# apple/swift-homomorphic-encryption

Measured on NVIDIA H100. Metric: BFV ct*ct mults/sec at N=8192, 4 coefficient moduli, higher is better.
Workload: dtype u64

## Files before the change

### swift-homomorphic-encryption_b200/csrc/context.cu

```cuda
#include "context.hpp"

#include <cuda_runtime.h>

#include <cmath>
#include <cstdlib>
#include <cstring>

#include "hostmath.hpp"
#include "ntt_fast.cuh"

namespace hecuda {
using namespace host;


static void fill_barrett(u64 p, u64 &mu1, u64 &mu_hi, u64 &mu_lo) {
    mu1 = (u64)(((u128)1 << 64) / p);
    u128 mu = (p & (p - 1)) == 0 ? ((u128)1 << (128 - (bit_length(p) - 1))) : (~(u128)0) / p;
    mu_hi = (u64)(mu >> 64);
    mu_lo = (u64)mu;
}

static bool build_slot(HostSlot &hs, u64 p, int64_t n, int logn, u64 t, u64 floor_w, std::vector<ulonglong2> &tw,
                       std::vector<ulonglong2> &itw, std::string &err) {
    if (!is_prime(p) || (p - 1) % (2 * (u64)n) != 0) {
// ... 99 lines not shown
    for (u64 qi : c->q)
        if (t >= qi) { err = "invalidEncryptionParameters: plaintext modulus must be below every coefficient modulus"; delete c; return nullptr; }
    c->bsk = smallest_ntt_primes(word_bits - 3, L + 1, (u64)n);
    if ((int)c->bsk.size() != L + 1) { err = "notEnoughPrimes for Bsk"; delete c; return nullptr; }
    for (u64 b : c->bsk)
        for (int i = 0; i < nmod; ++i)
            if (b == coeff_moduli[i]) { err = "coprimeModuli: coefficient modulus collides with the BEHZ base"; delete c; return nullptr; }

    c->aux = c->bsk;
    {
        const char *env = std::getenv("HECUDA_AUX_BASE");
        const bool want_fast = !(env && std::string(env) == "reference");
        const int widths[2] = {30, 55};
        double log_q = 0;
        for (u64 v : c->q) log_q += std::log2((double)v);
        const double log_n = (double)c->logn, log_t = std::log2((double)t);
        for (int wi = 0; wi < 2 && want_fast && c->aux == c->bsk && word_bits == 64; ++wi) {
            std::vector<u64> cand = widths[wi] == 55 ? smallest_ntt_primes(55, L + 1 + nmod, 1ull << 31)
                                                     : smallest_ntt_primes(widths[wi], L + 1 + nmod, (u64)n);
            std::vector<u64> pick;
            for (u64 v : cand) {
                bool used = false;
                for (int i = 0; i < nmod; ++i) used |= coeff_moduli[i] == v;
                if (!used && (int)pick.size() < L + 1) pick.push_back(v);
            }
            double log_aux = 0, log_aux_l = 0;
            for (size_t j = 0; j < pick.size(); ++j) {
                log_aux += std::log2((double)pick[j]);
                if ((int)j < L) log_aux_l += std::log2((double)pick[j]);
            }
            const bool enough = (int)pick.size() == L + 1 && log_aux >= log_q + log_n + 4 &&
                                log_aux_l + std::log2((double)pick.back()) >= log_t + log_n + log_q + 5;
            if (enough) c->aux = pick;
        }
    }
    c->aux_is_reference = c->aux == c->bsk;

    c->simd = is_prime(t) && (t - 1) % (2 * (u64)n) == 0;
    const int nslots = (c->aux_is_reference ? 2 * L + 2 : 3 * L + 3) + (c->simd ? 1 : 0);
    c->slots.resize(nslots);
    std::vector<u64> slot_mod(nslots);
    if (c->simd) slot_mod[c->slot_t()] = t;
    for (int i = 0; i < L; ++i) slot_mod[c->slot_q(i)] = c->q[i];
    for (int j = 0; j <= L; ++j) slot_mod[c->slot_bsk(j)] = c->bsk[j];
    slot_mod[c->slot_ks()] = c->q_ks;
    if (!c->aux_is_reference)
        for (int j = 0; j <= L; ++j) slot_mod[c->slot_aux(j)] = c->aux[j];
    const size_t table_bytes = sizeof(ulonglong2) * (size_t)n;
    const bool fast = c->logn >= fast::kMinLogN && c->logn <= fast::kMaxLogN;
    const bool split = c->logn == fast::kSplitLogN;
    const int half_logn = c->logn - 1;
    const int64_t half_n = n / 2;
    const int threads = (int)((split ? half_n : n) / 16);
    const size_t tr_bytes = (fast || split) ? sizeof(ulonglong2) * (size_t)15 * threads : 0;
    const size_t half_bytes = sizeof(ulonglong2) * (size_t)half_n;
    const size_t slot_bytes = 2 * table_bytes + (split ? 2 * (2 * half_bytes + 2 * tr_bytes) : 2 * tr_bytes);
    if (cudaMalloc(&c->d_pool, slot_bytes * nslots) != cudaSuccess) { err = "cudaMalloc failed for twiddle tables"; delete c; return nullptr; }
    std::vector<ulonglong2> tw, itw, tr(15 * (size_t)threads), itr(15 * (size_t)threads), twh, itwh;
    std::vector<ModSlot> dev_slots(split ? 3 * nslots : nslots);
    c->split_slot_base = split ? nslots : 0;
    for (int s = 0; s < nslots; ++s) {
        if (s == c->slot_ks() && !c->has_ks) {
            std::memset(&c->slots[s].dev, 0, sizeof(ModSlot));
            dev_slots[s] = c->slots[s].dev;
            continue;
        }
        const u64 floor_w = s < L ? invmod(punctured_mod(c->q.data(), L, s, slot_mod[s]), slot_mod[s]) : 1;
        if (!build_slot(c->slots[s], slot_mod[s], n, c->logn, t, floor_w, tw, itw, err)) { delete c; return nullptr; }
        char *base = (char *)c->d_pool + slot_bytes * s;
        cudaMemcpy(base, tw.data(), table_bytes, cudaMemcpyHostToDevice);
        cudaMemcpy(base + table_bytes, itw.data(), table_bytes, cudaMemcpyHostToDevice);
        c->slots[s].dev.tw = (const ulonglong2 *)base;
        c->slots[s].dev.itw = (const ulonglong2 *)(base + table_bytes);
        if (fast) {
            for (int k = 0; k < 15; ++k)
                for (int tau = 0; tau < threads; ++tau) {
                    tr[(size_t)k * threads + tau] = tw[fast::fwd_last_source(c->logn, k, tau)];
                    itr[(size_t)k * threads + tau] = itw[fast::inv_first_source(c->logn, k, tau)];
                }
            cudaMemcpy(base + 2 * table_bytes, tr.data(), tr_bytes, cudaMemcpyHostToDevice);
            cudaMemcpy(base + 2 * table_bytes + tr_bytes, itr.data(), tr_bytes, cudaMemcpyHostToDevice);
            c->slots[s].dev.tw_t = (const ulonglong2 *)(base + 2 * table_bytes);
            c->slots[s].dev.itw_t = (const ulonglong2 *)(base + 2 * table_bytes + tr_bytes);
        }
        dev_slots[s] = c->slots[s].dev;
        if (split) {
            for (int hh = 0; hh < 2; ++hh) {
                twh.assign(half_n, tw[0]);
                itwh.assign(half_n, itw[0]);
                for (int64_t i = 1; i < half_n; ++i) {
                    const int sp = bit_length((u64)i) - 1;
                    const int64_t src = ((int64_t)(2 + hh) << sp) + (i - ((int64_t)1 << sp));
                    twh[i] = tw[src];
                    itwh[i] = itw[src];
                }
                for (int k = 0; k < 15; ++k)
                    for (int tau = 0; tau < threads; ++tau) {
                        tr[(size_t)k * threads + tau] = twh[fast::fwd_last_source(half_logn, k, tau)];
                        itr[(size_t)k * threads + tau] = itwh[fast::inv_first_source(half_logn, k, tau)];
                    }
                char *hb = base + 2 * table_bytes + hh * (2 * half_bytes + 2 * tr_bytes);
                cudaMemcpy(hb, twh.data(), half_bytes, cudaMemcpyHostToDevice);
                cudaMemcpy(hb + half_bytes, itwh.data(), half_bytes, cudaMemcpyHostToDevice);
                cudaMemcpy(hb + 2 * half_bytes, tr.data(), tr_bytes, cudaMemcpyHostToDevice);
                cudaMemcpy(hb + 2 * half_bytes + tr_bytes, itr.data(), tr_bytes, cudaMemcpyHostToDevice);
                ModSlot v = c->slots[s].dev;
                v.tw = (const ulonglong2 *)hb;
                v.itw = (const ulonglong2 *)(hb + half_bytes);
                v.tw_t = (const ulonglong2 *)(hb + 2 * half_bytes);
                v.itw_t = (const ulonglong2 *)(hb + 2 * half_bytes + tr_bytes);
                dev_slots[nslots + 2 * s + hh] = v;
            }
        }
    }
    if (cudaMalloc(&c->d_slots, sizeof(ModSlot) * dev_slots.size()) != cudaSuccess) { err = "cudaMalloc failed"; delete c; return nullptr; }
    cudaMemcpy(c->d_slots, dev_slots.data(), sizeof(ModSlot) * dev_slots.size(), cudaMemcpyHostToDevice);

    const u64 *Q = c->q.data();
    auto build_behz = [&](const std::vector<u64> &base, bool reference_base, LiftConsts &lf, FloorConsts &fl) {
    const u64 *BSK = base.data();
    const u64 msk = base[L];
    auto slot_of = [&](int j) { return reference_base ? c->slot_bsk(j) : c->slot_aux(j); };
    std::memset(&lf, 0, sizeof(lf));
    lf.L = L;
    bool h_primes = true;
    for (int j = 0; j <= L; ++j) h_primes &= fast::class_of_modulus(BSK[j], bit_length(BSK[j])) == fast::kNarrowH;
    lf.h_primes = h_primes ? 1 : 0;
// ... 212 lines not shown
```

### swift-homomorphic-encryption_b200/csrc/context.hpp

```cpp
#pragma once
#include <cstdint>
#include <string>
#include <vector>

#include "modarith.cuh"

namespace hecuda {

constexpr int kMaxL = 32;
constexpr int kMaxSlots = 3 * kMaxL + 4;
constexpr int kMaxRows = 2 * kMaxL + 1;

struct ModSlot {
    u64 p;
    u64 mu1;
    u64 mu_hi, mu_lo;
    u64 mu_prod;
    int s_prod;
    int bits;
    int red_shift;
    u32 red_recip;
    u64 ninv;
    u64 r64;
    struct InvScale { u64 c0, c0p, c1, c1p; } inv_scale[4];
    const ulonglong2 *tw;
    const ulonglong2 *itw;
    const ulonglong2 *tw_t;
    const ulonglong2 *itw_t;
};

enum { kScalePlain = 0, kScaleTMont = 1, kScaleMont = 2, kScaleTMontFloor = 3 };

struct NttRowMap {
    int rows_per_poly;
    int group;
    unsigned char slot[kMaxRows + 1];
    int src_mod;
    long long src_poly_stride;
    unsigned char src_slot[kMaxRows + 1];
};

struct LiftConsts {
    int L;
    int wide_sums;
    u64 b_mu1[kMaxL + 1];
    u64 q[kMaxL];
    u64 in_w[kMaxL], in_wp[kMaxL];
    u32 punct_mt[kMaxL];
    u32 neg_inv_q_mt;
    u32 mt_mask, mt_half;
    u64 neg_off[kMaxL + 1];
    u64 b[kMaxL + 1], b_ninv[kMaxL + 1];
    u64 mat[kMaxL + 1][kMaxL];
    u64 qr[kMaxL + 1];
    int h_primes;
};

struct FloorConsts {
    int L;
    int wide_sums;
    u64 msk_mu1;
    u64 q[kMaxL], q_ninv[kMaxL], q_mu1[kMaxL];
    u64 inq_w[kMaxL], inq_wp[kMaxL];
    u64 b[kMaxL + 1], b_ninv[kMaxL + 1];
    u64 b_mu1[kMaxL + 1];
    u64 fq[kMaxL + 1];
    u64 fmat[kMaxL + 1][kMaxL];
    u64 amat[kMaxL];
    u64 a_msk;
    u64 omat[kMaxL][kMaxL];
    u64 b_mod_q[kMaxL], neg_b_mod_q[kMaxL];
    int h_primes;
};

struct DivRoundConsts {
    int l;
    u64 m[kMaxL + 1], mu1[kMaxL + 1];
    u64 last, half;
    u64 half_mod[kMaxL + 1];
    u64 inv_w[kMaxL + 1], inv_wp[kMaxL + 1];
};
// ... 65 lines not shown
```

### swift-homomorphic-encryption_b200/csrc/ntt_fast.cu

```cuda
#include <cuda.h>

#include <mutex>

#include <algorithm>
#include "kernels.cuh"
#include "ntt_fast.cuh"

namespace hecuda {
using namespace fast;

constexpr int kMaxRowList = 2 * (kMaxL + 1) * kMaxL;
struct RowList {
    int rows_per_poly;
    int count;
    unsigned short row[kMaxRowList];
    unsigned short slot[kMaxRowList];
    unsigned char flags[kMaxRowList];
    unsigned short src_row[kMaxRowList];
    long long src_poly_stride;
};

__device__ __forceinline__ u32 smem_u32(const void *p) { return (u32)__cvta_generic_to_shared(p); }
__device__ __forceinline__ void mbar_init(u64 *bar, int count) {
    asm volatile("mbarrier.init.shared::cta.b64 [%0], %1;" ::"r"(smem_u32(bar)), "r"(count) : "memory");
// ... 62 lines not shown
    }
    fwd_row_pass<LOGN, CLS, P - 1>(x, sm, tau, m, false);
}

template <int LOGN, int CLS, int K>
__device__ __forceinline__ void inv_row_pass(u64 (&x)[16], u64 *sm, int tau, const RowMod &m) {
    constexpr int C = inv_c(LOGN, K), LB = inv_lb(LOGN, K);
    load_smem<LOGN, LB, C>(x, sm, tau);
    if (narrow_like(CLS) && K > 0 && inv_reduce_at(LOGN, K)) inv_reduce(x, m);
    inv_pass<LOGN, LB, C, CLS, inv_bound_in(LOGN, K)>(x, tau, m);
    if (K == plan_passes(LOGN) - 1 && m.partial) {
        if (CLS == kSmall) {
#pragma unroll
            for (int r = 0; r < 16; ++r) x[r] = csub32((u32)x[r], (u32)(0 - m.np));
        } else {
            reduce_small16(x, m);
        }
    }
    store_smem<LOGN, LB, C>(x, sm, tau);
}
template <int LOGN, int CLS>
__device__ __forceinline__ void inv_row(u64 *sm, int tau, const RowMod &m) {
    constexpr int P = plan_passes(LOGN);
    u64 x[16];
    inv_row_pass<LOGN, CLS, 0>(x, sm, tau, m);
    __syncthreads();
    inv_row_pass<LOGN, CLS, 1>(x, sm, tau, m);
    __syncthreads();
    if (P == 4) {
        inv_row_pass<LOGN, CLS, (P == 4 ? 2 : 1)>(x, sm, tau, m);
        __syncthreads();
    }
    inv_row_pass<LOGN, CLS, P - 1>(x, sm, tau, m);
}

template <int LOGN, unsigned CLASSES>
__device__ __forceinline__ void fwd_row_of(int cls, u64 *sm, int tau, const RowMod &m, bool reduce_in) {
    if (has_class(CLASSES, kNarrowH) && cls == kNarrowH) fwd_row<LOGN, kNarrowH>(sm, tau, m, reduce_in);
    else if (has_class(CLASSES, kNarrow) && narrow_like(cls)) fwd_row<LOGN, kNarrow>(sm, tau, m, reduce_in);
    else if (has_class(CLASSES, kSmall) && cls == kSmall) fwd_row<LOGN, kSmall>(sm, tau, m, reduce_in);
    else if (has_class(CLASSES, kMid) && cls == kMid) fwd_row<LOGN, kMid>(sm, tau, m, reduce_in);
    else if (has_class(CLASSES, kWide)) fwd_row<LOGN, kWide>(sm, tau, m, reduce_in);
}
template <int LOGN, unsigned CLASSES>
__device__ __forceinline__ void inv_row_of(int cls, u64 *sm, int tau, const RowMod &m) {
    if (has_class(CLASSES, kNarrowH) && cls == kNarrowH) inv_row<LOGN, kNarrowH>(sm, tau, m);
    else if (has_class(CLASSES, kNarrow) && narrow_like(cls)) inv_row<LOGN, kNarrow>(sm, tau, m);
    else if (has_class(CLASSES, kSmall) && cls == kSmall) inv_row<LOGN, kSmall>(sm, tau, m);
    else if (has_class(CLASSES, kMid) && cls == kMid) inv_row<LOGN, kMid>(sm, tau, m);
    else if (has_class(CLASSES, kWide)) inv_row<LOGN, kWide>(sm, tau, m);
}

HE_HD constexpr int ntt_row_buffers(int logn) { return logn == 13 ? 2 : 1; }

template <int LOGN>
constexpr size_t ntt_smem_bytes() {
    constexpr int B = ntt_row_buffers(LOGN);
    return sizeof(u64) * B * ((size_t)1 << LOGN) + sizeof(ulonglong2) * ((size_t)1 << (LOGN - 4)) + sizeof(u64) * (B + 1);
}

constexpr int ntt_min_ctas(int logn) { return logn == 13 ? 1 : 1024 / ((1 << logn) / 16); }

template <int LOGN, bool INVERSE, unsigned CLASSES>
__global__ void __launch_bounds__((1 << LOGN) / 16, ntt_min_ctas(LOGN))
    ntt_rows_kernel(const __grid_constant__ CUtensorMap map_in, const __grid_constant__ CUtensorMap map_out,
                    const ModSlot *__restrict__ slots, const __grid_constant__ RowList rl, const int polys,
                    const int scale_mode) {
    extern __shared__ __align__(1024) u64 smem[];
    constexpr int kLines = (1 << LOGN) / kLineWords;
    constexpr int kBoxes = kLines > kBoxLines ? kLines / kBoxLines : 1;
    constexpr int kLinesPerBox = kLines / kBoxes;
    constexpr u32 kRowBytes = (u32)sizeof(u64) << LOGN, kTwBytes = (u32)sizeof(ulonglong2) << (LOGN - 4);
    constexpr int B = ntt_row_buffers(LOGN), AHEAD = B > 1 ? 1 : 0;
    ulonglong2 *tw_cache = reinterpret_cast<ulonglong2 *>(smem + B * (1 << LOGN));
    u64 *bar_row = reinterpret_cast<u64 *>(tw_cache + (1 << (LOGN - 4)));
    u64 *bar_tw = bar_row + B;
    const int tau = threadIdx.x;
    const int tasks = polys * rl.count;
    auto in_line = [&](int t) {
        const int w = t / polys, p = t - w * polys;
        const int64_t word = INVERSE ? ((int64_t)p * rl.rows_per_poly + rl.row[w]) << LOGN
                                     : (int64_t)p * rl.src_poly_stride + ((int64_t)rl.src_row[w] << LOGN);
        return (int)(word >> 4);
    };
    auto load_row = [&](int t, int buf) {
        mbar_arrive_expect_tx(&bar_row[buf], kRowBytes);
        const int line = in_line(t);
        u64 *dst = smem + buf * (1 << LOGN);
#pragma unroll
        for (int b = 0; b < kBoxes; ++b) tma_load_box(dst + b * kLinesPerBox * kLineWords, &map_in, line + b * kLinesPerBox, &bar_row[buf]);
    };
    if (tau == 0) {
        if (smem_u32(smem) & 1023) __trap();
#pragma unroll
        for (int b = 0; b < B; ++b) mbar_init(&bar_row[b], 1);
        mbar_init(bar_tw, 1);
        if (AHEAD && (int)blockIdx.x < tasks) load_row(blockIdx.x, 0);
    }
    __syncthreads();
    u32 phase_row = 0, phase_tw = 0;
    int cached_slot = -1;
    int buf = 0;
    for (int task = blockIdx.x; task < tasks; task += gridDim.x) {
        const int which = task / polys;
        const int poly = task - which * polys;
        const int flags = rl.flags[which];
        const int slot = rl.slot[which];
        const ModSlot &S = slots[slot];
        u64 *sm = smem + buf * (1 << LOGN);
        const int64_t out_word = ((int64_t)poly * rl.rows_per_poly + rl.row[which]) << LOGN;
        const bool new_slot = slot != cached_slot;
        cached_slot = slot;
        if (tau == 0) {
            if (new_slot) {
                mbar_arrive_expect_tx(bar_tw, kTwBytes);
                tma_load_1d(tw_cache, INVERSE ? S.itw : S.tw, kTwBytes, bar_tw);
            }
            const int fill = task + AHEAD * gridDim.x;
            if (fill < tasks) {
                tma_store_wait_read<B - 1 - AHEAD>();
                load_row(fill, (buf + AHEAD) % B);
            }
            const int next = fill + gridDim.x;
            if (next < tasks) {
                const int line = in_line(next);
#pragma unroll
                for (int b = 0; b < kBoxes; ++b) tma_prefetch_box(&map_in, line + b * kLinesPerBox);
            }
        }
        const int cls = flags & 7;
        RowMod m;
        m.np = 0 - S.p;
        m.kp = (cls == kWide || cls == kSmall) ? 2 * S.p : 4 * S.p;
        m.tw = nullptr;
        m.tw_s = smem_u32(tw_cache);
        m.slot = &S;
        m.scale_mode = INVERSE ? scale_mode : -1;
        m.partial = INVERSE && (flags & 16) != 0;
        if (new_slot) {
            mbar_wait(bar_tw, phase_tw);
            phase_tw ^= 1;
        }
        mbar_wait(&bar_row[buf], (phase_row >> buf) & 1);
        phase_row ^= 1u << buf;
        if (INVERSE) inv_row_of<LOGN, CLASSES>(cls, sm, tau, m);
        else fwd_row_of<LOGN, CLASSES>(cls, sm, tau, m, (flags & 8) != 0);
        fence_proxy_async_smem();
        __syncthreads();
        if (tau == 0) {
            const int line = (int)(out_word >> 4);
#pragma unroll
            for (int b = 0; b < kBoxes; ++b) tma_store_box(&map_out, line + b * kLinesPerBox, sm + b * kLinesPerBox * kLineWords);
            tma_commit();
        }
        buf = buf + 1 == B ? 0 : buf + 1;
    }
    if (tau == 0) tma_store_wait_all();
}

__device__ __forceinline__ u32 cluster_ctarank() {
    u32 r;
    asm("mov.u32 %0, %%cluster_ctarank;" : "=r"(r));
    return r;
}
__device__ __forceinline__ int cluster_id_x() {
    u32 r;
    asm("mov.u32 %0, %%clusterid.x;" : "=r"(r));
    return (int)r;
}
__device__ __forceinline__ int cluster_count_x() {
    u32 r;
    asm("mov.u32 %0, %%nclusterid.x;" : "=r"(r));
    return (int)r;
}
__device__ __forceinline__ void cluster_arrive() { asm volatile("barrier.cluster.arrive.release.aligned;" ::: "memory"); }
__device__ __forceinline__ void cluster_wait() { asm volatile("barrier.cluster.wait.acquire.aligned;" ::: "memory"); }
__device__ __forceinline__ void cluster_arrive_relaxed() { asm volatile("barrier.cluster.arrive.relaxed.aligned;" ::: "memory"); }
__device__ __forceinline__ u32 cluster_map(u32 addr, u32 rank) {
    u32 r;
    asm volatile("mapa.shared::cluster.u32 %0, %1, %2;" : "=r"(r) : "r"(addr), "r"(rank));
    return r;
}
__device__ __forceinline__ ulonglong2 ld_cluster_v2(u32 addr) {
    ulonglong2 v;
    asm volatile("ld.shared::cluster.v2.u64 {%0, %1}, [%2];" : "=l"(v.x), "=l"(v.y) : "r"(addr) : "memory");
    return v;
}
template <bool H>
__device__ __forceinline__ u64 mont_product(u64 a, u64 b, u64 p, u64 ninv) { return csub(mont_reduce_c<H>((u128)a * b, p, ninv), p); }

template <int LOGN>
constexpr size_t ntt_tensor_smem_bytes() {
    return sizeof(u64) * 2 * ((size_t)1 << LOGN) + sizeof(ulonglong2) * ((size_t)1 << (LOGN - 4)) + sizeof(u64) * 3;
}

template <int LOGN, bool H>
__device__ __forceinline__ void tensor_step(const u64 *x, const u64 *y, u64 *out, int64_t comp, u32 rank, int tau, u64 p, u64 ninv) {
    constexpr int N = 1 << LOGN, T = N / 16;
    u64 *own = out + (rank ? 2 * comp : 0);
#pragma unroll 4
    for (int w = 2 * tau; w < N; w += 2 * T) {
        const ulonglong2 a = *reinterpret_cast<const ulonglong2 *>(x + w), b = *reinterpret_cast<const ulonglong2 *>(y + w);
        *reinterpret_cast<ulonglong2 *>(own + smem_phys(w)) =
            make_ulonglong2(mont_product<H>(a.x, b.x, p, ninv), mont_product<H>(a.y, b.y, p, ninv));
    }
    cluster_wait();
    const u32 px = cluster_map(smem_u32(x), rank ^ 1), py = cluster_map(smem_u32(y), rank ^ 1);
#pragma unroll 4
    for (int w = (int)rank * (N / 2) + 2 * tau; w < ((int)rank + 1) * (N / 2); w += 2 * T) {
        const ulonglong2 a = *reinterpret_cast<const ulonglong2 *>(x + w), b = *reinterpret_cast<const ulonglong2 *>(y + w);
        const ulonglong2 A = ld_cluster_v2(px + 8u * w), Bv = ld_cluster_v2(py + 8u * w);
        u128 m0 = (u128)a.x * Bv.x, m1 = (u128)a.y * Bv.y;
        mac128(m0, A.x, b.x);
        mac128(m1, A.y, b.y);
        *reinterpret_cast<ulonglong2 *>(out + comp + smem_phys(w)) =
            make_ulonglong2(csub(mont_reduce_c<H>(m0, p, ninv), p), csub(mont_reduce_c<H>(m1, p, ninv), p));
    }
}

template <int LOGN, unsigned CLASSES>
__global__ void __launch_bounds__((1 << LOGN) / 16, 1)
    ntt_forward_tensor_kernel(const __grid_constant__ CUtensorMap map_lhs, const __grid_constant__ CUtensorMap map_rhs,
                              const __grid_constant__ CUtensorMap map_ext, u64 *__restrict__ ten,
                              const ModSlot *__restrict__ slots, const __grid_constant__ RowList rl, const int items,
                              const int L) {
    extern __shared__ __align__(1024) u64 smem[];
    constexpr int N = 1 << LOGN;
    constexpr int kBoxes = N / kLineWords / kBoxLines;
    constexpr u32 kRowBytes = (u32)sizeof(u64) << LOGN, kTwBytes = (u32)sizeof(ulonglong2) << (LOGN - 4);
    static_assert(kBoxes >= 1, "one row is at least one box");
    ulonglong2 *tw_cache = reinterpret_cast<ulonglong2 *>(smem + 2 * N);
    u64 *bar_row = reinterpret_cast<u64 *>(tw_cache + N / 16);
    u64 *bar_tw = bar_row + 2;
    const int tau = threadIdx.x;
    const u32 rank = cluster_ctarank();
    const int first = cluster_id_x(), stride = cluster_count_x();
    const int R = rl.rows_per_poly;
    const int tasks = items * rl.count;
    auto load_row = [&](int t, int j) {
        const int w = t / items, item = t - w * items, r = rl.row[w];
        const CUtensorMap *map;
        int64_t word;
        if (r < L) {
            map = j ? &map_rhs : &map_lhs;
            word = ((int64_t)(2 * item + (int)rank) * L + r) << LOGN;
        } else {
            map = &map_ext;
            word = ((int64_t)(4 * item + 2 * j + (int)rank) * (L + 1) + r - L) << LOGN;
        }
        const int line = (int)(word >> 4);
        mbar_arrive_expect_tx(&bar_row[j], kRowBytes);
#pragma unroll
        for (int b = 0; b < kBoxes; ++b) tma_load_box(smem + j * N + b * kBoxLines * kLineWords, map, line + b * kBoxLines, &bar_row[j]);
    };
    if (tau == 0) {
        if (smem_u32(smem) & 1023) __trap();
        mbar_init(&bar_row[0], 1);
        mbar_init(&bar_row[1], 1);
        mbar_init(bar_tw, 1);
    }
    cluster_arrive();
    cluster_wait();
    u32 phase_row = 0, phase_tw = 0;
    int cached_slot = -1;
    for (int task = first; task < tasks; task += stride) {
        if (task != first) cluster_wait();
        const int which = task / items;
        const int item = task - which * items;
        const int slot = rl.slot[which], r = rl.row[which], cls = rl.flags[which] & 7;
        const ModSlot &S = slots[slot];
        const bool new_slot = slot != cached_slot;
        cached_slot = slot;
        if (tau == 0) {
            if (new_slot) {
                mbar_arrive_expect_tx(bar_tw, kTwBytes);
                tma_load_1d(tw_cache, S.tw, kTwBytes, bar_tw);
            }
            load_row(task, 0);
            load_row(task, 1);
        }
        RowMod m;
        m.np = 0 - S.p;
        m.kp = (cls == kWide || cls == kSmall) ? 2 * S.p : 4 * S.p;
        m.tw = nullptr;
        m.tw_s = smem_u32(tw_cache);
        m.slot = &S;
        m.scale_mode = -1;
        m.partial = false;
        if (new_slot) {
            mbar_wait(bar_tw, phase_tw);
            phase_tw ^= 1;
        }
#pragma unroll
        for (int j = 0; j < 2; ++j) {
            mbar_wait(&bar_row[j], phase_row);
            fwd_row_of<LOGN, CLASSES>(cls, smem + j * N, tau, m, false);
        }
        phase_row ^= 1;
        __syncthreads();
        cluster_arrive();
        const int64_t comp = (int64_t)R * N;
        u64 *out = ten + ((int64_t)3 * item * R + r) * N;
        if (has_class(CLASSES, kNarrowH) && cls == kNarrowH) tensor_step<LOGN, true>(smem, smem + N, out, comp, rank, tau, S.p, S.ninv);
        else tensor_step<LOGN, false>(smem, smem + N, out, comp, rank, tau, S.p, S.ninv);
        fence_proxy_async_smem();
        cluster_arrive_relaxed();
    }
    if (first < tasks) cluster_wait();
}

static void build_row_list(const Context &ctx, const NttRowMap &map, bool inverse, RowList &rl) {
    rl.rows_per_poly = map.rows_per_poly;
    rl.count = 0;
    rl.src_poly_stride = map.src_mod ? map.src_poly_stride : (long long)map.rows_per_poly * ctx.n;
    static const int order[5] = {kWide, kMid, kNarrow, kNarrowH, kSmall};
    for (int oi = 0; oi < 5; ++oi) {
        const int cls = order[oi];
        for (int r = 0; r < map.rows_per_poly; ++r) {
            const int slot = map.slot[r / map.group];
            if (class_of_modulus(ctx.slots[slot].dev.p, ctx.slots[slot].dev.bits) != cls) continue;
            const int i = rl.count++;
            rl.row[i] = (unsigned short)r;
            rl.slot[i] = (unsigned short)slot;
            rl.src_row[i] = (unsigned short)(map.src_mod && !inverse ? r % map.src_mod : r);
            int flags = cls;
            if (map.src_mod && !inverse) {
                const u64 p = ctx.slots[slot].dev.p, src_p = ctx.slots[map.src_slot[r % map.src_mod]].dev.p;
                const u64 room = narrow_like(cls) ? 2u : cls == kMid ? 8u : cls == kSmall ? 1u : 4u;
                if (src_p > p && (src_p - 1) / p >= room) flags |= 8;
// ... 267 lines not shown
```

### swift-homomorphic-encryption_b200/csrc/ntt_fast.cuh

```cuda
#pragma once
#include "context.hpp"
#include "modarith.cuh"

namespace hecuda {
namespace fast {

constexpr int kMinLogN = 10, kMaxLogN = 14;
constexpr int kSplitLogN = 15;
constexpr int kNarrowBits = 55;
constexpr int kMidBits = 61;
constexpr int kSmallBits = 30;
enum { kNarrow = 0, kMid = 1, kWide = 2, kSmall = 3, kNarrowH = 4 };
HE_HD constexpr int class_of_bits(int bits) {
    return bits <= kSmallBits ? kSmall : bits <= kNarrowBits ? kNarrow : bits <= kMidBits ? kMid : kWide;
}
HE_HD constexpr int class_of_modulus(u64 p, int bits) {
    return (class_of_bits(bits) == kNarrow && (u32)p == 1u) ? kNarrowH : class_of_bits(bits);
}
HE_HD constexpr bool narrow_like(int cls) { return cls == kNarrow || cls == kNarrowH; }

HE_HD constexpr unsigned class_bit(int cls) { return 1u << cls; }
constexpr unsigned kAllClasses = (1u << kNarrow) | (1u << kMid) | (1u << kWide) | (1u << kSmall);
constexpr unsigned kNarrowClasses = (1u << kNarrow) | (1u << kNarrowH);
HE_HD constexpr bool has_class(unsigned set, int cls) { return (set & class_bit(cls)) != 0; }
// ... 74 lines not shown
}
template <int LB, int C>
HE_HD constexpr int reg_offset(int r) {
    return ((r >> pass_e(LB, C)) << LB) | (r & ((1 << pass_e(LB, C)) - 1));
}
template <int LB, int C>
HE_HD constexpr bool pass_vec() { return pass_e(LB, C) >= 1 || LB == 0; }

template <int LB, int C>
HE_HD int reg_word(int base_phys, int r) {
    constexpr int kSwizzled = 0x7e;
    const int off = reg_offset<LB, C>(r);
    return (off & kSwizzled) ? (base_phys ^ smem_phys(off)) : (base_phys + off);
}

template <int LOGN, int LB, int C>
HE_HD void load_smem(u64 (&x)[16], const u64 *sm, int tau) {
    const int b = smem_phys(elem_index<LOGN, LB, C>(tau, 0));
    if (pass_vec<LB, C>()) {
#pragma unroll
        for (int r = 0; r < 16; r += 2) {
            const ulonglong2 v = *reinterpret_cast<const ulonglong2 *>(sm + reg_word<LB, C>(b, r));
            x[r] = v.x;
            x[r + 1] = v.y;
        }
    } else {
#pragma unroll
        for (int r = 0; r < 16; ++r) x[r] = sm[reg_word<LB, C>(b, r)];
    }
}
template <int LOGN, int LB, int C>
HE_HD void store_smem(const u64 (&x)[16], u64 *sm, int tau) {
    const int b = smem_phys(elem_index<LOGN, LB, C>(tau, 0));
    if (pass_vec<LB, C>()) {
#pragma unroll
        for (int r = 0; r < 16; r += 2)
            *reinterpret_cast<ulonglong2 *>(sm + reg_word<LB, C>(b, r)) = make_ulonglong2(x[r], x[r + 1]);
    } else {
#pragma unroll
        for (int r = 0; r < 16; ++r) sm[reg_word<LB, C>(b, r)] = x[r];
    }
}

struct RowMod {
    u64 np;
    u64 kp;
    const ulonglong2 *tw;
    unsigned tw_s;
    const ModSlot *slot;
    int scale_mode;
    bool partial;
    HE_HD const ulonglong2 *tw_t() const { return scale_mode < 0 ? slot->tw_t : slot->itw_t; }
};
HE_HD ulonglong2 ld_tw_cached(const RowMod &m, int index) {
#if defined(__CUDA_ARCH__)
    ulonglong2 v;
    asm volatile("ld.shared.v2.u64 {%0, %1}, [%2];" : "=l"(v.x), "=l"(v.y) : "r"(m.tw_s + (unsigned)index * 16u));
    return v;
#else
    return m.tw[index];
#endif
}
HE_HD u64 ld_u64(const u64 *p) {
#if defined(__CUDA_ARCH__)
    return __ldg(p);
#else
    return *p;
#endif
}

HE_HD u64 pack64(u32 lo, u32 hi) {
#if defined(__CUDA_ARCH__)
    u64 v;
    asm("mov.b64 %0, {%1, %2};" : "=l"(v) : "r"(lo), "r"(hi));
    return v;
#else
    return ((u64)hi << 32) | lo;
#endif
}
HE_HD void unpack64(u64 v, u32 &lo, u32 &hi) {
#if defined(__CUDA_ARCH__)
    asm("mov.b64 {%0, %1}, %2;" : "=r"(lo), "=r"(hi) : "l"(v));
#else
    lo = (u32)v;
    hi = (u32)(v >> 32);
#endif
}
HE_HD u64 mul_wide_u32(u32 a, u32 b) {
#if defined(__CUDA_ARCH__)
    u64 d;
    asm("mul.wide.u32 %0, %1, %2;" : "=l"(d) : "r"(a), "r"(b));
    return d;
#else
    return (u64)a * b;
#endif
}
HE_HD u64 mad_wide_u32(u32 a, u32 b, u64 c) {
#if defined(__CUDA_ARCH__)
    u64 d;
    asm("mad.wide.u32 %0, %1, %2, %3;" : "=l"(d) : "r"(a), "r"(b), "l"(c));
    return d;
#else
    return (u64)a * b + c;
#endif
}
HE_HD u32 mul_hi_u32(u32 a, u32 b) {
#if defined(__CUDA_ARCH__)
    return __umulhi(a, b);
#else
    return (u32)(((u64)a * b) >> 32);
#endif
}

// ... 49 lines not shown
        "mov.b64 A, {a1, z};\n\t"
        "mov.b64 B, {b1, z};\n\t"
        "mad.wide.u32 Q, y1, p1, A;\n\t"
        "add.u64 Q, Q, B;\n\t"
        "mov.b64 {q0, q1}, Q;\n\t"
        "mul.wide.u32 V, y0, w0;\n\t"
        "mov.b64 {v0, v1}, V;\n\t"
        "mad.lo.u32 v1, y1, w0, v1;\n\t"
        "mad.lo.u32 v1, y0, w1, v1;\n\t"
        "mad.lo.u32 v1, q0, nh, v1;\n\t"
        "sub.cc.u32 v0, v0, q0;\n\t"
        "subc.u32 v1, v1, q1;\n\t"
        "mov.b64 %0, {v0, v1};\n\t}"
        : "=l"(v)
        : "l"(y), "l"(w), "l"(wp), "l"(np));
    return v;
#else
    const u32 y0 = (u32)y, y1 = (u32)(y >> 32), wp0 = (u32)wp, wp1 = (u32)(wp >> 32);
    const u64 q = (u64)y1 * wp1 + (((u64)y1 * wp0) >> 32) + (((u64)y0 * wp1) >> 32);
    const u64 h = (0 - np) >> 32;
    return y * w - q - ((u64)((u32)q * (u32)h) << 32);
#endif
}
template <int CLS>
HE_HD u64 shoup4c(u64 y, u64 w, u64 wp, u64 np) { return CLS == kNarrowH ? shoup4h(y, w, wp, np) : shoup4(y, w, wp, np); }
HE_HD u64 shoup2(u64 y, u64 w, u64 wp, u64 np) { return y * w + mulhi64(y, wp) * np; }

HE_HD u64 reduce_small(u64 x, const u64 p, const u64 np, const int red_shift, const u32 red_recip) {
    const u32 xs = (u32)(x >> red_shift);
    const u32 qhat = mul_hi_u32(xs, red_recip);
    u32 np0, np1, rl, rh;
    unpack64(np, np0, np1);
    unpack64(mad_wide_u32(qhat, np0, x), rl, rh);
    rh = qhat * np1 + rh;
    return csub(pack64(rl, rh), p);
}
HE_HD void reduce_small16(u64 (&x)[16], const RowMod &m) {
    const int shift = m.slot->red_shift;
    const u32 recip = m.slot->red_recip;
    const u64 p = 0 - m.np;
#pragma unroll
    for (int r = 0; r < 16; ++r) x[r] = reduce_small(x[r], p, m.np, shift, recip);
}

HE_HD u32 csub32(u32 x, u32 m) {
    const u32 d = x - m;
    return d < x ? d : x;
}
HE_HD u32 shoup32(u32 y, u32 w, u32 wp, u32 p) {
    return y * w - mul_hi_u32(y, wp) * p;
}

template <int CLS>
HE_HD void ct_butterfly(u64 &x, u64 &y, const ulonglong2 w, const RowMod &m) {
    if (CLS == kSmall) {
        const u32 p = (u32)(0 - m.np), p2 = 2 * p;
        const u32 xr = csub32((u32)x, p2);
        const u32 v = shoup32((u32)y, (u32)w.x, (u32)(w.y >> 32), p);
        x = xr + v;
        y = xr - v + p2;
    } else if (narrow_like(CLS)) {
        const u64 v = shoup4c<CLS>(y, w.x, w.y, m.np);
        const u64 xo = x + v;
        y = x - v + m.kp;
        x = xo;
    } else if (CLS == kMid) {
        const u64 xr = csub(x, m.kp);
        const u64 v = shoup4(y, w.x, w.y, m.np);
        x = xr + v;
        y = xr - v + m.kp;
    } else {
        const u64 xr = csub(x, m.kp);
        const u64 v = shoup2(y, w.x, w.y, m.np);
        x = xr + v;
        y = xr - v + m.kp;
    }
}

template <int LOGN, int LB, int C, int CLS, int J>
HE_HD void fwd_stage(u64 (&x)[16], int tau, const RowMod &m) {
    constexpr int E = pass_e(LB, C), F = 1 << E, S0 = LOGN - LB - C, T = (1 << LOGN) / 16;
    constexpr int H = 1 << (C - 1 - J);
    const int hi = tau >> (LB - E);
    const ulonglong2 *tw_t = LB == 0 ? m.tw_t() + tau : nullptr;
#pragma unroll
    for (int grp = 0; grp < (1 << J); ++grp) {
        const ulonglong2 w = LB == 0 ? ld_tw(tw_t + ((1 << J) - 1 + grp) * T)
                                     : ld_tw_cached(m, (1 << (S0 + J)) + (hi << J) + grp);
#pragma unroll
        for (int k = 0; k < H; ++k) {
            const int a = grp * 2 * H + k;
#pragma unroll
            for (int f = 0; f < F; ++f) ct_butterfly<CLS>(x[a * F + f], x[(a + H) * F + f], w, m);
        }
    }
}
template <int LOGN, int LB, int C, int CLS>
HE_HD void fwd_pass(u64 (&x)[16], int tau, const RowMod &m) {
    fwd_stage<LOGN, LB, C, CLS, 0>(x, tau, m);
    if (C > 1) fwd_stage<LOGN, LB, C, CLS, (C > 1 ? 1 : 0)>(x, tau, m);
    if (C > 2) fwd_stage<LOGN, LB, C, CLS, (C > 2 ? 2 : 0)>(x, tau, m);
    if (C > 3) fwd_stage<LOGN, LB, C, CLS, (C > 3 ? 3 : 0)>(x, tau, m);
}

template <int CLS>
HE_HD void fwd_finish(u64 (&x)[16], const RowMod &m) {
    if (CLS == kSmall) {
        const u32 p = (u32)(0 - m.np);
#pragma unroll
        for (int r = 0; r < 16; ++r) x[r] = csub32(csub32((u32)x[r], 2 * p), p);
    } else {
        reduce_small16(x, m);
    }
}

template <int CLS>
HE_HD void gs_butterfly(u64 &x, u64 &y, const ulonglong2 w, const RowMod &m, u64 kp) {
    if (CLS == kSmall) {
        const u32 p = (u32)(0 - m.np), p2 = 2 * p;
        const u32 s = csub32((u32)x + (u32)y, p2);
        y = shoup32((u32)x - (u32)y + p2, (u32)w.x, (u32)(w.y >> 32), p);
        x = s;
    } else if (narrow_like(CLS)) {
        const u64 s = x + y;
        y = shoup4c<CLS>(x - y + kp, w.x, w.y, m.np);
        x = s;
    } else if (CLS == kMid) {
        const u64 s = csub(x + y, kp);
        y = shoup4(x - y + kp, w.x, w.y, m.np);
        x = s;
    } else {
        const u64 s = csub(x + y, kp);
        y = shoup2(x - y + kp, w.x, w.y, m.np);
        x = s;
    }
}

template <int LOGN, int LB, int C, int CLS, int BIN, int J>
HE_HD void inv_stage(u64 (&x)[16], const int tau, const RowMod &m) {
    constexpr int E = pass_e(LB, C), F = 1 << E, T = (1 << LOGN) / 16;
    constexpr int HH = 1 << J;
    constexpr bool kLast = (LB + J == LOGN - 1);
    constexpr int kGroups = 1 << (LOGN - 1 - LB - J);
    const int hi = tau >> (LB - E);
    const u64 kp = narrow_like(CLS) ? (0 - m.np) * (u64)inv_bound_after(BIN, J) : m.kp;
    const ulonglong2 *tw_t = LB == 0 ? m.tw_t() + tau : nullptr;
#pragma unroll
    for (int grp = 0; grp < (1 << (C - 1 - J)); ++grp) {
        if (!kLast || m.partial) {
            const ulonglong2 w = LB == 0 ? ld_tw(tw_t + (16 - (16 >> J) + grp) * T)
                                         : ld_tw_cached(m, kGroups + (hi << (C - 1 - J)) + grp);
#pragma unroll
            for (int k = 0; k < HH; ++k) {
                const int a = grp * 2 * HH + k;
#pragma unroll
                for (int f = 0; f < F; ++f) gs_butterfly<CLS>(x[a * F + f], x[(a + HH) * F + f], w, m, kp);
            }
        } else {
            const u64 *sc = &m.slot->inv_scale[m.scale_mode].c0;
            const u64 c0 = ld_u64(sc), c0p = ld_u64(sc + 1), c1 = ld_u64(sc + 2), c1p = ld_u64(sc + 3);
#pragma unroll
            for (int k = 0; k < HH; ++k) {
                const int a = grp * 2 * HH + k;
#pragma unroll
                for (int f = 0; f < F; ++f) {
                    if (CLS == kSmall) {
                        const u32 p = (u32)(0 - m.np);
                        const u32 xa = (u32)x[a * F + f], ya = (u32)x[(a + HH) * F + f];
                        x[a * F + f] = csub32(shoup32(xa + ya, (u32)c0, (u32)(c0p >> 32), p), p);
                        x[(a + HH) * F + f] = csub32(shoup32(xa - ya + 2 * p, (u32)c1, (u32)(c1p >> 32), p), p);
                        continue;
                    }
                    const u64 xa = x[a * F + f], ya = x[(a + HH) * F + f];
                    const u64 s = xa + ya;
                    const u64 d = xa - ya + kp;
                    x[a * F + f] = csub(shoup2(s, c0, c0p, m.np), 0 - m.np);
                    x[(a + HH) * F + f] = csub(shoup2(d, c1, c1p, m.np), 0 - m.np);
                }
            }
        }
    }
}

template <int LOGN, int LB, int C, int CLS, int BIN>
HE_HD void inv_pass(u64 (&x)[16], int tau, const RowMod &m) {
    inv_stage<LOGN, LB, C, CLS, BIN, 0>(x, tau, m);
    if (C > 1) inv_stage<LOGN, LB, C, CLS, BIN, (C > 1 ? 1 : 0)>(x, tau, m);
    if (C > 2) inv_stage<LOGN, LB, C, CLS, BIN, (C > 2 ? 2 : 0)>(x, tau, m);
    if (C > 3) inv_stage<LOGN, LB, C, CLS, BIN, (C > 3 ? 3 : 0)>(x, tau, m);
}

HE_HD void inv_reduce(u64 (&x)[16], const RowMod &m) { reduce_small16(x, m); }

HE_HD int fwd_last_source(int logn, int k, int tau) {
    int j = 0;
    while ((2 << j) - 1 <= k) ++j;
    const int grp = k - ((1 << j) - 1);
    return (1 << (logn - 4 + j)) + (tau << j) + grp;
}
HE_HD int inv_first_source(int logn, int k, int tau) {
    int J = 0;
    while (16 - (16 >> (J + 1)) <= k) ++J;
    const int grp = k - (16 - (16 >> J));
    return (1 << (logn - 1 - J)) + (tau << (3 - J)) + grp;
}

}
}
```

Measured before the change: 151,500.

## Keep last-pass NTT twiddles resident in shared memory for N=8192

For logn 13 the per-slot twiddle image now covers the thread-specific twiddles of the final forward and first inverse radix-16 pass. The whole image is bulk-loaded into shared memory by TMA, replacing scattered global loads of 15 per-thread twiddles. To fit the 227 KB shared memory budget, only 11 of the 15 are stored. The remaining odd groups are rebuilt by multiplying by the primitive root, which adds one modular multiply per affected butterfly and a host-side check that the table is in bit-reversed order.

```diff
diff --git a/swift-homomorphic-encryption_b200/csrc/context.cu b/swift-homomorphic-encryption_b200/csrc/context.cu
--- a/swift-homomorphic-encryption_b200/csrc/context.cu
+++ b/swift-homomorphic-encryption_b200/csrc/context.cu
@@ -175,9 +175,11 @@
     const int half_logn = c->logn - 1;
     const int64_t half_n = n / 2;
     const int threads = (int)((split ? half_n : n) / 16);
-    const size_t tr_bytes = (fast || split) ? sizeof(ulonglong2) * (size_t)15 * threads : 0;
+    const bool resident = fast && fast::resident_twiddles(c->logn);
+    const size_t tr_bytes = (fast || split) && !resident ? sizeof(ulonglong2) * (size_t)15 * threads : 0;
+    const size_t img_bytes = resident ? sizeof(ulonglong2) * (size_t)fast::image_entries(c->logn) : 0;
     const size_t half_bytes = sizeof(ulonglong2) * (size_t)half_n;
-    const size_t slot_bytes = 2 * table_bytes + (split ? 2 * (2 * half_bytes + 2 * tr_bytes) : 2 * tr_bytes);
+    const size_t slot_bytes = 2 * table_bytes + (split ? 2 * (2 * half_bytes + 2 * tr_bytes) : 2 * tr_bytes + 2 * img_bytes);
     if (cudaMalloc(&c->d_pool, slot_bytes * nslots) != cudaSuccess) { err = "cudaMalloc failed for twiddle tables"; delete c; return nullptr; }
     std::vector<ulonglong2> tw, itw, tr(15 * (size_t)threads), itr(15 * (size_t)threads), twh, itwh;
     std::vector<ModSlot> dev_slots(split ? 3 * nslots : nslots);
@@ -195,7 +197,25 @@
         cudaMemcpy(base + table_bytes, itw.data(), table_bytes, cudaMemcpyHostToDevice);
         c->slots[s].dev.tw = (const ulonglong2 *)base;
         c->slots[s].dev.itw = (const ulonglong2 *)(base + table_bytes);
-        if (fast) {
+        if (resident) {
+            const u64 p = slot_mod[s];
+            for (int64_t i = n / 2 + 1; i < n; i += 2)
+                if (tw[i].x != mulmod(tw[i - 1].x, tw[1].x, p) || itw[i].x != mulmod(itw[i - 1].x, itw[1].x, p)) {
+                    err = "internal error: twiddle table of " + std::to_string(p) + " is not in bit-reversed order";
+                    delete c;
+                    return nullptr;
+                }
+            const int entries = fast::image_entries(c->logn);
+            std::vector<ulonglong2> img(entries), iimg(entries);
+            for (int i = 0; i < entries; ++i) {
+                img[i] = tw[fast::image_source(c->logn, false, i)];
+                iimg[i] = itw[fast::image_source(c->logn, true, i)];
+            }
+            cudaMemcpy(base + 2 * table_bytes, img.data(), img_bytes, cudaMemcpyHostToDevice);
+            cudaMemcpy(base + 2 * table_bytes + img_bytes, iimg.data(), img_bytes, cudaMemcpyHostToDevice);
+            c->slots[s].dev.tw_img = (const ulonglong2 *)(base + 2 * table_bytes);
+            c->slots[s].dev.itw_img = (const ulonglong2 *)(base + 2 * table_bytes + img_bytes);
+        } else if (fast) {
             for (int k = 0; k < 15; ++k)
                 for (int tau = 0; tau < threads; ++tau) {
                     tr[(size_t)k * threads + tau] = tw[fast::fwd_last_source(c->logn, k, tau)];
diff --git a/swift-homomorphic-encryption_b200/csrc/context.hpp b/swift-homomorphic-encryption_b200/csrc/context.hpp
--- a/swift-homomorphic-encryption_b200/csrc/context.hpp
+++ b/swift-homomorphic-encryption_b200/csrc/context.hpp
@@ -27,6 +27,8 @@
     const ulonglong2 *itw;
     const ulonglong2 *tw_t;
     const ulonglong2 *itw_t;
+    const ulonglong2 *tw_img;
+    const ulonglong2 *itw_img;
 };
 
 enum { kScalePlain = 0, kScaleTMont = 1, kScaleMont = 2, kScaleTMontFloor = 3 };
diff --git a/swift-homomorphic-encryption_b200/csrc/ntt_fast.cu b/swift-homomorphic-encryption_b200/csrc/ntt_fast.cu
--- a/swift-homomorphic-encryption_b200/csrc/ntt_fast.cu
+++ b/swift-homomorphic-encryption_b200/csrc/ntt_fast.cu
@@ -138,12 +138,24 @@
 }
 
 HE_HD constexpr int ntt_row_buffers(int logn) { return logn == 13 ? 2 : 1; }
+template <int LOGN>
+HE_HD constexpr u32 ntt_twiddle_bytes() {
+    return (u32)sizeof(ulonglong2) * (resident_twiddles(LOGN) ? image_entries(LOGN) : 1 << (LOGN - 4));
+}
+static_assert(ntt_twiddle_bytes<13>() == 98304 && ntt_twiddle_bytes<13>() % 16 == 0 && ntt_twiddle_bytes<13>() < (1u << 20),
+              "the resident image is one 1-D bulk copy on one mbarrier");
+template <int LOGN, bool INVERSE>
+__device__ __forceinline__ const ulonglong2 *ntt_twiddle_source(const ModSlot &S) {
+    if (resident_twiddles(LOGN)) return INVERSE ? S.itw_img : S.tw_img;
+    return INVERSE ? S.itw : S.tw;
+}
 
 template <int LOGN>
 constexpr size_t ntt_smem_bytes() {
     constexpr int B = ntt_row_buffers(LOGN);
-    return sizeof(u64) * B * ((size_t)1 << LOGN) + sizeof(ulonglong2) * ((size_t)1 << (LOGN - 4)) + sizeof(u64) * (B + 1);
-}
+    return sizeof(u64) * B * ((size_t)1 << LOGN) + ntt_twiddle_bytes<LOGN>() + sizeof(u64) * (B + 1);
+}
+static_assert(ntt_smem_bytes<13>() == 229400 && ntt_smem_bytes<13>() <= 232448, "N = 2^13: 227 KB of shared memory a CTA");
 
 constexpr int ntt_min_ctas(int logn) { return logn == 13 ? 1 : 1024 / ((1 << logn) / 16); }
 
@@ -156,10 +168,10 @@
     constexpr int kLines = (1 << LOGN) / kLineWords;
     constexpr int kBoxes = kLines > kBoxLines ? kLines / kBoxLines : 1;
     constexpr int kLinesPerBox = kLines / kBoxes;
-    constexpr u32 kRowBytes = (u32)sizeof(u64) << LOGN, kTwBytes = (u32)sizeof(ulonglong2) << (LOGN - 4);
+    constexpr u32 kRowBytes = (u32)sizeof(u64) << LOGN, kTwBytes = ntt_twiddle_bytes<LOGN>();
     constexpr int B = ntt_row_buffers(LOGN), AHEAD = B > 1 ? 1 : 0;
     ulonglong2 *tw_cache = reinterpret_cast<ulonglong2 *>(smem + B * (1 << LOGN));
-    u64 *bar_row = reinterpret_cast<u64 *>(tw_cache + (1 << (LOGN - 4)));
+    u64 *bar_row = reinterpret_cast<u64 *>(tw_cache + kTwBytes / sizeof(ulonglong2));
     u64 *bar_tw = bar_row + B;
     const int tau = threadIdx.x;
     const int tasks = polys * rl.count;
@@ -200,7 +212,7 @@
         if (tau == 0) {
             if (new_slot) {
                 mbar_arrive_expect_tx(bar_tw, kTwBytes);
-                tma_load_1d(tw_cache, INVERSE ? S.itw : S.tw, kTwBytes, bar_tw);
+                tma_load_1d(tw_cache, ntt_twiddle_source<LOGN, INVERSE>(S), kTwBytes, bar_tw);
             }
             const int fill = task + AHEAD * gridDim.x;
             if (fill < tasks) {
@@ -277,8 +289,9 @@
 
 template <int LOGN>
 constexpr size_t ntt_tensor_smem_bytes() {
-    return sizeof(u64) * 2 * ((size_t)1 << LOGN) + sizeof(ulonglong2) * ((size_t)1 << (LOGN - 4)) + sizeof(u64) * 3;
-}
+    return sizeof(u64) * 2 * ((size_t)1 << LOGN) + ntt_twiddle_bytes<LOGN>() + sizeof(u64) * 3;
+}
+static_assert(ntt_tensor_smem_bytes<13>() == 229400, "N = 2^13: 227 KB of shared memory a CTA");
 
 template <int LOGN, bool H>
 __device__ __forceinline__ void tensor_step(const u64 *x, const u64 *y, u64 *out, int64_t comp, u32 rank, int tau, u64 p, u64 ninv) {
@@ -313,10 +326,10 @@
     extern __shared__ __align__(1024) u64 smem[];
     constexpr int N = 1 << LOGN;
     constexpr int kBoxes = N / kLineWords / kBoxLines;
-    constexpr u32 kRowBytes = (u32)sizeof(u64) << LOGN, kTwBytes = (u32)sizeof(ulonglong2) << (LOGN - 4);
+    constexpr u32 kRowBytes = (u32)sizeof(u64) << LOGN, kTwBytes = ntt_twiddle_bytes<LOGN>();
     static_assert(kBoxes >= 1, "one row is at least one box");
     ulonglong2 *tw_cache = reinterpret_cast<ulonglong2 *>(smem + 2 * N);
-    u64 *bar_row = reinterpret_cast<u64 *>(tw_cache + N / 16);
+    u64 *bar_row = reinterpret_cast<u64 *>(tw_cache + kTwBytes / sizeof(ulonglong2));
     u64 *bar_tw = bar_row + 2;
     const int tau = threadIdx.x;
     const u32 rank = cluster_ctarank();
@@ -360,7 +373,7 @@
         if (tau == 0) {
             if (new_slot) {
                 mbar_arrive_expect_tx(bar_tw, kTwBytes);
-                tma_load_1d(tw_cache, S.tw, kTwBytes, bar_tw);
+                tma_load_1d(tw_cache, ntt_twiddle_source<LOGN, false>(S), kTwBytes, bar_tw);
             }
             load_row(task, 0);
             load_row(task, 1);
diff --git a/swift-homomorphic-encryption_b200/csrc/ntt_fast.cuh b/swift-homomorphic-encryption_b200/csrc/ntt_fast.cuh
--- a/swift-homomorphic-encryption_b200/csrc/ntt_fast.cuh
+++ b/swift-homomorphic-encryption_b200/csrc/ntt_fast.cuh
@@ -150,6 +150,13 @@
     bool partial;
     HE_HD const ulonglong2 *tw_t() const { return scale_mode < 0 ? slot->tw_t : slot->itw_t; }
 };
+
+HE_HD constexpr bool resident_twiddles(int logn) { return logn == 13; }
+constexpr int kImageSlots = 11;
+HE_HD constexpr int image_entries(int logn) { return (1 << (logn - 4)) * (1 + kImageSlots); }
+HE_HD constexpr int fwd_image_k(int kp) { return kp < 7 ? kp : 7 + 2 * (kp - 7); }
+HE_HD constexpr int inv_image_k(int kp) { return kp < 4 ? 2 * kp : kp + 4; }
+
 HE_HD ulonglong2 ld_tw_cached(const RowMod &m, int index) {
 #if defined(__CUDA_ARCH__)
     ulonglong2 v;
@@ -157,6 +164,13 @@
     return v;
 #else
     return m.tw[index];
+#endif
+}
+HE_HD ulonglong2 ld_tw_image(const RowMod &m, int kp, int tau, int T) {
+#if defined(__CUDA_ARCH__)
+    return ld_tw_cached(m, T + kp * T + tau);
+#else
+    return m.tw_t()[(m.scale_mode < 0 ? fwd_image_k(kp) : inv_image_k(kp)) * T + tau];
 #endif
 }
 HE_HD u64 ld_u64(const u64 *p) {
@@ -312,6 +326,14 @@
 }
 
 template <int CLS>
+HE_HD u64 tw_mul(u64 y, const ulonglong2 w, const RowMod &m) {
+    if (CLS == kSmall) return shoup32((u32)y, (u32)w.x, (u32)(w.y >> 32), (u32)(0 - m.np));
+    if (narrow_like(CLS)) return shoup4c<CLS>(y, w.x, w.y, m.np);
+    if (CLS == kMid) return shoup4(y, w.x, w.y, m.np);
+    return shoup2(y, w.x, w.y, m.np);
+}
+
+template <int CLS>
 HE_HD void ct_butterfly(u64 &x, u64 &y, const ulonglong2 w, const RowMod &m) {
     if (CLS == kSmall) {
         const u32 p = (u32)(0 - m.np), p2 = 2 * p;
@@ -341,17 +363,27 @@
 HE_HD void fwd_stage(u64 (&x)[16], int tau, const RowMod &m) {
     constexpr int E = pass_e(LB, C), F = 1 << E, S0 = LOGN - LB - C, T = (1 << LOGN) / 16;
     constexpr int H = 1 << (C - 1 - J);
+    constexpr bool kImage = LB == 0 && resident_twiddles(LOGN);
+    constexpr bool kZeta = kImage && J == 3;
     const int hi = tau >> (LB - E);
-    const ulonglong2 *tw_t = LB == 0 ? m.tw_t() + tau : nullptr;
+    const ulonglong2 *tw_t = LB == 0 && !kImage ? m.tw_t() + tau : nullptr;
+    const ulonglong2 zeta = kZeta ? ld_tw_cached(m, 1) : make_ulonglong2(0, 0);
+    ulonglong2 w = make_ulonglong2(0, 0);
 #pragma unroll
     for (int grp = 0; grp < (1 << J); ++grp) {
-        const ulonglong2 w = LB == 0 ? ld_tw(tw_t + ((1 << J) - 1 + grp) * T)
-                                     : ld_tw_cached(m, (1 << (S0 + J)) + (hi << J) + grp);
+        const bool odd = kZeta && (grp & 1);
+        if (!odd)
+            w = kImage  ? ld_tw_image(m, kZeta ? 7 + grp / 2 : (1 << J) - 1 + grp, tau, T)
+                : LB == 0 ? ld_tw(tw_t + ((1 << J) - 1 + grp) * T)
+                          : ld_tw_cached(m, (1 << (S0 + J)) + (hi << J) + grp);
 #pragma unroll
         for (int k = 0; k < H; ++k) {
             const int a = grp * 2 * H + k;
 #pragma unroll
-            for (int f = 0; f < F; ++f) ct_butterfly<CLS>(x[a * F + f], x[(a + H) * F + f], w, m);
+            for (int f = 0; f < F; ++f) {
+                if (odd) x[(a + H) * F + f] = tw_mul<CLS>(x[(a + H) * F + f], zeta, m);
+                ct_butterfly<CLS>(x[a * F + f], x[(a + H) * F + f], w, m);
+            }
         }
     }
 }
@@ -375,23 +407,31 @@
 }
 
 template <int CLS>
-HE_HD void gs_butterfly(u64 &x, u64 &y, const ulonglong2 w, const RowMod &m, u64 kp) {
+HE_HD void gs_butterfly(u64 &x, u64 &y, const ulonglong2 w, const RowMod &m, u64 kp, const ulonglong2 *zeta = nullptr) {
     if (CLS == kSmall) {
         const u32 p = (u32)(0 - m.np), p2 = 2 * p;
         const u32 s = csub32((u32)x + (u32)y, p2);
-        y = shoup32((u32)x - (u32)y + p2, (u32)w.x, (u32)(w.y >> 32), p);
+        u32 d = (u32)x - (u32)y + p2;
+        if (zeta) d = (u32)tw_mul<CLS>(d, *zeta, m);
+        y = shoup32(d, (u32)w.x, (u32)(w.y >> 32), p);
         x = s;
     } else if (narrow_like(CLS)) {
         const u64 s = x + y;
-        y = shoup4c<CLS>(x - y + kp, w.x, w.y, m.np);
+        u64 d = x - y + kp;
+        if (zeta) d = tw_mul<CLS>(d, *zeta, m);
+        y = shoup4c<CLS>(d, w.x, w.y, m.np);
         x = s;
     } else if (CLS == kMid) {
         const u64 s = csub(x + y, kp);
-        y = shoup4(x - y + kp, w.x, w.y, m.np);
+        u64 d = x - y + kp;
+        if (zeta) d = tw_mul<CLS>(d, *zeta, m);
+        y = shoup4(d, w.x, w.y, m.np);
         x = s;
     } else {
         const u64 s = csub(x + y, kp);
-        y = shoup2(x - y + kp, w.x, w.y, m.np);
+        u64 d = x - y + kp;
+        if (zeta) d = tw_mul<CLS>(d, *zeta, m);
+        y = shoup2(d, w.x, w.y, m.np);
         x = s;
     }
 }
@@ -404,17 +444,24 @@
     constexpr int kGroups = 1 << (LOGN - 1 - LB - J);
     const int hi = tau >> (LB - E);
     const u64 kp = narrow_like(CLS) ? (0 - m.np) * (u64)inv_bound_after(BIN, J) : m.kp;
-    const ulonglong2 *tw_t = LB == 0 ? m.tw_t() + tau : nullptr;
+    constexpr bool kImage = LB == 0 && resident_twiddles(LOGN);
+    constexpr bool kZeta = kImage && J == 0;
+    const ulonglong2 *tw_t = LB == 0 && !kImage ? m.tw_t() + tau : nullptr;
+    const ulonglong2 zeta = kZeta ? ld_tw_cached(m, 1) : make_ulonglong2(0, 0);
+    ulonglong2 w = make_ulonglong2(0, 0);
 #pragma unroll
     for (int grp = 0; grp < (1 << (C - 1 - J)); ++grp) {
         if (!kLast || m.partial) {
-            const ulonglong2 w = LB == 0 ? ld_tw(tw_t + (16 - (16 >> J) + grp) * T)
-                                         : ld_tw_cached(m, kGroups + (hi << (C - 1 - J)) + grp);
+            const bool odd = kZeta && (grp & 1);
+            if (!odd)
+                w = kImage  ? ld_tw_image(m, kZeta ? grp / 2 : 16 - (16 >> J) + grp - 4, tau, T)
+                    : LB == 0 ? ld_tw(tw_t + (16 - (16 >> J) + grp) * T)
+                              : ld_tw_cached(m, kGroups + (hi << (C - 1 - J)) + grp);
 #pragma unroll
             for (int k = 0; k < HH; ++k) {
                 const int a = grp * 2 * HH + k;
 #pragma unroll
-                for (int f = 0; f < F; ++f) gs_butterfly<CLS>(x[a * F + f], x[(a + HH) * F + f], w, m, kp);
+                for (int f = 0; f < F; ++f) gs_butterfly<CLS>(x[a * F + f], x[(a + HH) * F + f], w, m, kp, odd ? &zeta : nullptr);
             }
         } else {
             const u64 *sc = &m.slot->inv_scale[m.scale_mode].c0;
@@ -464,6 +511,12 @@
     const int grp = k - (16 - (16 >> J));
     return (1 << (logn - 1 - J)) + (tau << (3 - J)) + grp;
 }
-
-}
-}
+HE_HD int image_source(int logn, bool inverse, int i) {
+    const int T = 1 << (logn - 4);
+    if (i < T) return i;
+    const int kp = i / T - 1, tau = i % T;
+    return inverse ? inv_first_source(logn, inv_image_k(kp), tau) : fwd_last_source(logn, fwd_image_k(kp), tau);
+}
+
+}
+}
```

Result: faster. 158,200, median of 6 (+4.4%).
